# openai/blocksparse

Measured on AMD Instinct MI355X. Metric: bsmm_effective_tflops_4096x4096_bs32_d20, higher is better.
Workload: dtype bf16

## Files before the change

### blocksparse_amd/csrc/bsmm_updat_v2.h

```cpp
#pragma once
#include <type_traits>

#include "bsmm_common.h"
#include "bsmm_plan.h"
#include "bsmm_updat_tr.h"

namespace bsmm {

#ifndef U2_NT_PARTS
#define U2_NT_PARTS 1
#endif
#ifndef U2_MAX_SLICES
#define U2_MAX_SLICES 8
#endif
#ifndef U2_CH_ROWS
#define U2_CH_ROWS 16
#endif
#ifndef U2_SETB_FROM
#define U2_SETB_FROM 0
#endif
constexpr int U2_CH = U2_CH_ROWS;
constexpr int U2_KS = U2_CH / 16;
constexpr int U2_D = 64 / U2_CH;
constexpr int U2_AHEAD = U2_D / 2;
static_assert(U2_CH == 16 || U2_CH == 32, "chunk = 1 or 2 K-steps");
constexpr int u2_ring(int ws) { return ws == 32 ? 2 : U2_D; }
constexpr int u2_lds_bytes(int ws) { return u2_ring(ws) * 2 * U2_CH * ws * 64; }
constexpr int U2_CH0 = 32;
#ifndef U2_RING5
#define U2_RING5 0
#endif
constexpr int u2_lds_bytes0(int ws) { return U2_RING5 ? 5 * ws * 32 * (U2_CH0 * 2) : 131072; }

#ifdef U2_STAMPS
__device__ unsigned long long g_u2_trace[1024 * 8];
#define U2_STAMP(k, v) do { if (wave == 0 && lane == 0 && blockIdx.x < 1024) g_u2_trace[blockIdx.x * 8 + (k)] = (v); } while (0)
#else
#define U2_STAMP(k, v) do { } while (0)
#endif

__device__ __forceinline__ const void* uniform_ptr(const void* p) {
    const uint64_t v = reinterpret_cast<uint64_t>(p);
    const uint32_t lo = __builtin_amdgcn_readfirstlane((uint32_t)v), hi = __builtin_amdgcn_readfirstlane((uint32_t)(v >> 32));
    return reinterpret_cast<const void*>(((uint64_t)hi << 32) | lo);
}

__device__ __forceinline__ void glds16_saddr(const void* sbase, uint32_t voff, uint32_t lds_byte_addr) {
    unsigned keep;
    asm volatile("s_mov_b32 %0, m0\n\ts_mov_b32 m0, %3\n\ts_nop 0\n\tglobal_load_lds_dwordx4 %1, %2\n\ts_mov_b32 m0, %0"
                 : "=&s"(keep)
                 : "v"(voff), "s"(sbase), "s"(lds_byte_addr)
                 : "memory");
}
__device__ __forceinline__ void glds16_saddr_x2(const void* sbase, uint32_t voff0, uint32_t voff1, uint32_t lds_byte_addr) {
    unsigned keep;
    asm volatile("s_mov_b32 %0, m0\n\ts_mov_b32 m0, %4\n\ts_nop 0\n\tglobal_load_lds_dwordx4 %1, %3\n\t"
                 "s_add_u32 m0, m0, 0x400\n\ts_nop 0\n\tglobal_load_lds_dwordx4 %2, %3\n\ts_mov_b32 m0, %0"
                 : "=&s"(keep)
                 : "v"(voff0), "v"(voff1), "s"(sbase), "s"(lds_byte_addr)
                 : "memory", "scc");
}

__device__ __forceinline__ void glds16_saddr_x4(const void* sbase, uint32_t v0, uint32_t v1, uint32_t v2, uint32_t v3, uint32_t lds_byte_addr) {
    unsigned keep;
    asm volatile("s_mov_b32 %0, m0\n\ts_mov_b32 m0, %6\n\ts_nop 0\n\tglobal_load_lds_dwordx4 %1, %5\n\t"
                 "s_add_u32 m0, m0, 0x400\n\ts_nop 0\n\tglobal_load_lds_dwordx4 %2, %5\n\t"
                 "s_add_u32 m0, m0, 0x400\n\ts_nop 0\n\tglobal_load_lds_dwordx4 %3, %5\n\t"
                 "s_add_u32 m0, m0, 0x400\n\ts_nop 0\n\tglobal_load_lds_dwordx4 %4, %5\n\ts_mov_b32 m0, %0"
                 : "=&s"(keep)
                 : "v"(v0), "v"(v1), "v"(v2), "v"(v3), "s"(sbase), "s"(lds_byte_addr)
                 : "memory", "scc");
}

__device__ __forceinline__ const unsigned char* pick_ptr(const PtrList8& l, int idx) {
    const void* p = l.p[0];
#pragma unroll
    for (int k = 1; k < 8; ++k) p = (idx == k) ? l.p[k] : p;
    return static_cast<const unsigned char*>(p);
}

template <class DT, int LDSB>
__device__ __forceinline__ void u2_direct_block(const PtrList8& Xs, const PtrList8& Es, float* __restrict__ scratch, const int32_t* __restrict__ plan,
                                                int N, int Cf, int Kf, int pcount, int e, long region0, unsigned char* smem) {
    typedef typename DT::T T;
    constexpr int SLOT = 2048, D = LDSB / U2_WAVES / SLOT;
    static_assert(D >= 2 && LDSB >= U2_WAVES * 4096, "direct blocks: a ring of two chunks per wave and 64 KiB for the reduction");
    const int lane = threadIdx.x & 63;
    const int wave = __builtin_amdgcn_readfirstlane(threadIdx.x >> 6);
    const int DP = plan[30];
    const int d = e / DP, q = e - d * DP;
    const int32_t* de = plan + plan[29] + 4 * d;
    const int c = __builtin_amdgcn_readfirstlane(de[1]), k = __builtin_amdgcn_readfirstlane(de[2]);
    unsigned char* ring = smem + wave * (D * SLOT);
    const uint32_t ring_addr = lds_addr_of(ring);
    const int drow = lane >> 2, dpiece = lane & 3;
    const int g16 = lane >> 4, t16 = lane & 15, h = g16 >> 1;
    const int rd_base = (8 * h + (t16 >> 2)) * 64 + (16 * (g16 & 1) + 4 * (t16 & 3)) * 2;
    f32x16 acc;
#pragma unroll
    for (int i = 0; i < 16; ++i) acc[i] = 0.f;
    const int nch = (N + 15) >> 4;
    const int lo = (int)((long)nch * q / DP), hi = (int)((long)nch * (q + 1) / DP);
    const int first = lo + wave;
    const int myq = hi > first ? (hi - first + U2_WAVES - 1) / U2_WAVES : 0;
    for (int p = 0; p < pcount; ++p) {
        const T* X = reinterpret_cast<const T*>(pick_ptr(Xs, p)) + c * 32 + dpiece * 8;
        const T* E = reinterpret_cast<const T*>(pick_ptr(Es, p)) + k * 32 + dpiece * 8;
        auto issue = [&](int j, int pos) {
            const int r = min((first + U2_WAVES * j) * 16 + drow, N - 1);
            const uint32_t slot = __builtin_amdgcn_readfirstlane(ring_addr + pos * SLOT);
            glds16_asm(X + (size_t)r * Cf, slot);
            glds16_asm(E + (size_t)r * Kf, slot + 1024);
        };
#pragma unroll
        for (int j = 0; j < D - 1; ++j) issue(j, j);
        int rd_pos = 0, wr_pos = D - 1;
        for (int j = 0; j < myq; ++j) {
            issue(j + D - 1, wr_pos);
            asm volatile("s_waitcnt vmcnt(%0)" ::"n"(2 * (D - 1)) : "memory");
            const unsigned char* sp = ring + rd_pos * SLOT + rd_base;
            rd_pos = (rd_pos + 1 == D) ? 0 : rd_pos + 1;
            wr_pos = (wr_pos + 1 == D) ? 0 : wr_pos + 1;
            const uint2 a0 = ds_tr16(sp), a1 = ds_tr16(sp + 4 * 64), b0 = ds_tr16(sp + 1024), b1 = ds_tr16(sp + 1024 + 4 * 64);
            uint4 a = make_uint4(a0.x, a0.y, a1.x, a1.y);
            const uint4 b = make_uint4(b0.x, b0.y, b1.x, b1.y);
            const int nb = (first + U2_WAVES * j) * 16 + 8 * h;
            if (nb + 8 > N) {
                uint32_t* u = reinterpret_cast<uint32_t*>(&a);
#pragma unroll
                for (int i = 0; i < 4; ++i) u[i] &= ((nb + 2 * i < N) ? 0xffffu : 0u) | ((nb + 2 * i + 1 < N) ? 0xffff0000u : 0u);
            }
            asm volatile("s_waitcnt lgkmcnt(0)" ::: "memory");
            acc = DT::mfma32(a, b, acc);
        }
        asm volatile("s_waitcnt vmcnt(0)" ::: "memory");
    }
    __syncthreads();
    float* red = reinterpret_cast<float*>(smem);
#pragma unroll
    for (int reg = 0; reg < 16; ++reg) red[wave * 1024 + reg * 64 + lane] = acc[reg];
    __syncthreads();
    float sum = 0.f;
#pragma unroll
    for (int v = 0; v < U2_WAVES; ++v) sum += red[v * 1024 + threadIdx.x];
    const int reg = threadIdx.x >> 6, ln = threadIdx.x & 63;
    float* region = scratch + ((size_t)region0 * (U2_WAVES * U2_SLOTS) + (size_t)e) * 1024;
    region[((reg >> 2) * 64 + ln) * 4 + (reg & 3)] = sum;
}

template <class DT, int WS, int AXIS = 1>
__global__ void __launch_bounds__(64 * U2_WAVES, 4)
updat32_a1_v2_kernel(PtrList8 Xs, PtrList8 Es, typename DT::T* __restrict__ DW, float* __restrict__ scratch,
                     const int32_t* __restrict__ plan, int N, int Cf, int Kf, int pcount, float alpha, float beta, int flat, int main_grid, int rounds) {
    typedef typename DT::T T;
    static_assert(DT::is16 && (WS == 8 || WS == 16 || (WS == 32 && AXIS == 1)), "updat v2: 16-bit storage types, 8x8 / 16x16 windows (32x32: feature axis 1)");
    extern __shared__ __attribute__((aligned(16))) unsigned char smem[];
    constexpr int CH = AXIS == 1 ? U2_CH : U2_CH0;
    constexpr int KS = CH / 16;
    constexpr bool FIVE = AXIS == 0 && U2_RING5;
    constexpr int D = AXIS == 1 ? u2_ring(WS) : (WS == 16 ? 2 : 4);
    constexpr int AHEAD = D / 2;
    constexpr int ROWB = AXIS == 1 ? WS * 64 : CH * 2;
    constexpr int SLAB = AXIS == 1 ? CH * ROWB : WS * 32 * ROWB;
    constexpr int SLOT = 2 * SLAB;
    constexpr int PPR = ROWB / 16;
    constexpr int RPI = ROWB <= 1024 ? 1024 / ROWB : 1;
    constexpr int IPR = ROWB <= 1024 ? 1 : ROWB / 1024;
    constexpr int IPO = SLAB / 1024;
    constexpr int NI = 2 * IPO / U2_WAVES;
    static_assert((NI == 1 || NI == 2 || NI == 4) && NI * U2_WAVES == 2 * IPO && IPO % NI == 0, "the chunk must split evenly over the waves");

    const int mg = main_grid > 0 ? main_grid : (int)gridDim.x;
    if ((int)blockIdx.x >= mg) {
        if constexpr (AXIS == 1) u2_direct_block<DT, u2_lds_bytes(WS)>(Xs, Es, scratch, plan, N, Cf, Kf, pcount, (int)blockIdx.x - mg, (long)rounds * mg, smem);
        return;
    }
    const int lane = threadIdx.x & 63;
    const int wave = __builtin_amdgcn_readfirstlane(threadIdx.x >> 6);
    const int32_t* items = plan + plan[6];
    const int nchunks = (N + CH - 1) / CH;
    const int nfull = N / CH;
    const int CPI = pcount * nchunks;
    const bool xcd_mode = flat == 0 && (mg & 7) == 0;
    const int nsets = xcd_mode ? plan[8] : 1;
    const int nparts = xcd_mode ? 8 / nsets : 1;
    const int U = xcd_mode ? mg >> 3 : mg;
    const int xcd = xcd_mode ? (blockIdx.x & 7) : 0, uj = xcd_mode ? (blockIdx.x >> 3) : blockIdx.x;
    const int set = xcd / nparts, part = xcd - set * nparts;
    const int set_first = xcd_mode ? plan[9 + 2 * set] : 0, set_count = xcd_mode ? plan[10 + 2 * set] : plan[4];
    const int part_lo = (int)((long)part * CPI / nparts), part_hi = (int)((long)(part + 1) * CPI / nparts);
    const int full_rounds = set_count / U, m_last = set_count - full_rounds * U;
    const int k_last = m_last > 0 ? min(U / m_last, U2_MAX_SLICES) : 0;
    const int total_rounds = full_rounds + ((m_last > 0 && uj < m_last * k_last) ? 1 : 0);

    const uint32_t base_addr = lds_addr_of(smem);
    const int opE = (NI * wave) / IPO;
    const int ii0 = (NI * wave) % IPO;
    const int d_row0 = ROWB <= 1024 ? ii0 * RPI + lane / PPR : ii0 / IPR;
    auto row_of = [&](int q) -> int { return ROWB <= 1024 ? d_row0 + q * RPI : (ii0 + q) / IPR; };
    auto pos_of = [&](int q) -> int { return ROWB <= 1024 ? lane % PPR : ((ii0 + q) % IPR) * 64 + lane; };
    const uint32_t sub_off = ii0 * 1024;
    const uint32_t wave_off = (!FIVE ? opE * SLAB : 0) + sub_off;
    constexpr uint32_t HS = SLAB, RING0 = 5 * SLAB;
    const int F = opE ? Kf : Cf;
    const int my_piece0 = (lane % PPR) ^ ((d_row0 >> 2) & 3);
    const int g16 = lane >> 4, t16 = lane & 15;
    const int h = AXIS == 1 ? g16 >> 1 : lane >> 5;
    const int trow = t16 >> 2;
    const int tsub = (2 * (g16 & 1) + ((t16 & 3) >> 1)) * 16 + (t16 & 1) * 8;
    const int frag_row = AXIS == 1 ? (8 * h + trow) * ROWB + tsub : (lane & 31) * ROWB + ((h ^ (((lane & 31) >> 2) & 3)) << 4);
#ifdef U2_NO_PINGPONG
    const bool setb = false;
#else
    constexpr int SB = U2_SETB_FROM > 0 ? U2_SETB_FROM : ((WS == 8 && AXIS == 1) ? 4 : U2_WAVES / 2);
    const bool setb = wave >= SB;
#endif

    U2_STAMP(0, __builtin_amdgcn_s_memrealtime());
    U2_STAMP(4, (unsigned long long)total_rounds);
    for (int round = 0; round < total_rounds; ++round) {
        int item, r0, cnt;
        if (round < full_rounds) {
            item = set_first + round * U + uj;
            r0 = part_lo; cnt = part_hi - part_lo;
        } else {
            const int which = uj / k_last, slice = uj - which * k_last, L = part_hi - part_lo;
            item = set_first + full_rounds * U + which;
            r0 = part_lo + (int)((long)slice * L / k_last);
            cnt = part_lo + (int)((long)(slice + 1) * L / k_last) - r0;
        }
        if (cnt <= 0) continue;
        item = __builtin_amdgcn_readfirstlane(item);
        r0 = __builtin_amdgcn_readfirstlane(r0);
        cnt = __builtin_amdgcn_readfirstlane(cnt);
        const int32_t* it = items + (size_t)item * U2_ITEM;
        const int c0 = it[0], k0 = it[1];
        const int32_t* wd = it + 4 + wave * U2_WWORDS;
        const uint32_t meta = (uint32_t)__builtin_amdgcn_readfirstlane(wd[0]);
        const int n0 = meta & 15, n1 = (meta >> 4) & 15;

        auto piece_off = [&](int q) {
            const int row = row_of(q);
            if constexpr (AXIS == 1) {
                const int piece = pos_of(q) ^ (4 * (row & 3));
                const int col = min((opE ? k0 : c0) * 32 + piece * 8, F - 8);
                return (uint32_t)(row * F + col) * 2u;
            } else {
                const int piece = (lane % PPR) ^ ((row >> 2) & 3);
                const int feat = min((opE ? k0 : c0) * 32 + row, F - 1);
                return ((uint32_t)feat * (uint32_t)N + (uint32_t)piece * 8u) * 2u;
            }
        };
        const uint32_t voff0 = piece_off(0), voff1 = NI > 1 ? piece_off(1) : 0u, voff2 = NI > 2 ? piece_off(2) : 0u, voff3 = NI > 2 ? piece_off(3) : 0u;
        int aoff[2], boff[U2_SLOTS];
        if constexpr (AXIS == 1) {
            int c0i = (meta >> 8) & 15, c1i = (meta >> 12) & 15;
            if constexpr (WS == 32) {
                c0i |= (__builtin_amdgcn_readfirstlane(wd[1]) >> 29 & 1) << 4;
                c1i |= n1 > 0 ? (__builtin_amdgcn_readfirstlane(wd[1 + n0]) >> 29 & 1) << 4 : 0;
            }
            aoff[0] = frag_row + ((c0i ^ trow) << 6);
            aoff[1] = frag_row + ((c1i ^ trow) << 6);
#pragma unroll
            for (int j = 0; j < U2_SLOTS; ++j) {
                int ki = (meta >> (16 + 4 * j)) & 15;
                if constexpr (WS == 32) ki |= (__builtin_amdgcn_readfirstlane(wd[1 + j]) >> 30 & 1) << 4;
                boff[j] = SLAB + frag_row + ((ki ^ trow) << 6);
            }
        } else {
            aoff[0] = frag_row + (int)((meta >> 8) & 15) * (32 * ROWB);
            aoff[1] = frag_row + (int)((meta >> 12) & 15) * (32 * ROWB);
#pragma unroll
            for (int j = 0; j < U2_SLOTS; ++j) boff[j] = (FIVE ? 0 : SLAB) + frag_row + (int)((meta >> (16 + 4 * j)) & 15) * (32 * ROWB);
        }

        f32x16 acc[U2_SLOTS];
#pragma unroll
        for (int j = 0; j < U2_SLOTS; ++j)
#pragma unroll
            for (int i = 0; i < 16; ++i) acc[j][i] = 0.f;

        const uint32_t fstride = AXIS == 1 ? (uint32_t)(CH * F) * 2u : (uint32_t)CH * 2u;
        auto run = [&](auto n0_tag, auto n1_tag, auto setb_tag) {
            constexpr int N0 = decltype(n0_tag)::value, N1 = decltype(n1_tag)::value;
            constexpr bool SETB = decltype(setb_tag)::value;
            uint4 a0 = zero_u4(), a1 = zero_u4(), b[(N0 + N1) ? (N0 + N1) : 1];
#pragma unroll
            for (int j = 0; j < N0 + N1; ++j) b[j] = zero_u4();
            auto read_frags = [&](const unsigned char* slot, const unsigned char* slot_y, int ks) {
#ifdef U2_NO_READS
                asm volatile("" ::"s"(slot));
                return;
#endif
                if constexpr (AXIS == 1) {
                    slot += ks * 16 * ROWB;
                    {
                        const uint2 lo = ds_tr16(slot + aoff[0]), hi = ds_tr16(slot + aoff[0] + 4 * ROWB);
                        a0 = make_uint4(lo.x, lo.y, hi.x, hi.y);
                    }
                    if constexpr (N1 > 0) {
                        const uint2 lo = ds_tr16(slot + aoff[1]), hi = ds_tr16(slot + aoff[1] + 4 * ROWB);
                        a1 = make_uint4(lo.x, lo.y, hi.x, hi.y);
                    }
#pragma unroll
                    for (int j = 0; j < N0 + N1; ++j) {
                        const uint2 lo = ds_tr16(slot + boff[j]), hi = ds_tr16(slot + boff[j] + 4 * ROWB);
                        b[j] = make_uint4(lo.x, lo.y, hi.x, hi.y);
                    }
                } else {
                    a0 = *reinterpret_cast<const uint4*>(slot + (aoff[0] ^ (ks << 5)));
                    if constexpr (N1 > 0) a1 = *reinterpret_cast<const uint4*>(slot + (aoff[1] ^ (ks << 5)));
#pragma unroll
                    for (int j = 0; j < N0 + N1; ++j) b[j] = *reinterpret_cast<const uint4*>(slot_y + (boff[j] ^ (ks << 5)));
                }
            };
            auto multiply = [&]() {
#ifndef U2_NO_MFMA
#pragma unroll
                for (int j = 0; j < N0; ++j) acc[j] = DT::mfma32(a0, b[j], acc[j]);
                if constexpr (N1 > 0) {
#pragma unroll
                    for (int j = 0; j < N1; ++j) acc[N0 + j] = DT::mfma32(a1, b[N0 + j], acc[N0 + j]);
                }
#else
#pragma unroll
                for (int j = 0; j < N0 + N1; ++j) asm volatile("" ::"v"(b[j].x), "v"(b[j].y), "v"(b[j].z), "v"(b[j].w));
                asm volatile("" ::"v"(a0.x), "v"(a0.y), "v"(a0.z), "v"(a0.w));
                if constexpr (N1 > 0) asm volatile("" ::"v"(a1.x), "v"(a1.y), "v"(a1.z), "v"(a1.w));
#endif
            };
            const unsigned char* fb = nullptr;
            uint32_t rv0 = 0, rv1 = 0, rv2 = 0, rv3 = 0;
            int reg_left = 0, k_issue = 0;
#define U2_ISSUE_SLOW()                                                                                                      \
    do {                                                                                                                     \
        const int kk_ = min(k_issue, cnt - 1);                                                                               \
        const int g_ = r0 + kk_, p_ = __builtin_amdgcn_readfirstlane(g_ / nchunks), q_ = g_ - p_ * nchunks;                  \
        fb = static_cast<const unsigned char*>(uniform_ptr(opE ? pick_ptr(Es, p_) : pick_ptr(Xs, p_)));                      \
        const uint32_t dst_ = __builtin_amdgcn_readfirstlane(base_addr + wave_off + (!FIVE ? (uint32_t)(k_issue & (D - 1)) * SLOT : (uint32_t)((2 * k_issue + opE) % 5) * HS)); \
        uint32_t row_off_, sub0_, sub1_, sub2_, sub3_;                                                                       \
        if constexpr (AXIS == 1) {                                                        \
            row_off_ = (uint32_t)(q_ * CH * F) * 2u;                                                                         \
            sub0_ = (uint32_t)(max(0, q_ * CH + row_of(0) - (N - 1)) * F) * 2u;                                              \
            sub1_ = (uint32_t)(max(0, q_ * CH + row_of(1) - (N - 1)) * F) * 2u;                                              \
            sub2_ = (uint32_t)(max(0, q_ * CH + row_of(2) - (N - 1)) * F) * 2u;                                              \
            sub3_ = (uint32_t)(max(0, q_ * CH + row_of(3) - (N - 1)) * F) * 2u;                                              \
        } else {                                       \
            row_off_ = (uint32_t)(q_ * CH) * 2u;                                                                             \
            sub0_ = sub1_ = sub2_ = sub3_ = (uint32_t)max(0, q_ * CH + my_piece0 * 8 + 8 - N) * 2u;                          \
        }                                                                                                                    \
        U2_DMA1(fb, voff0 + row_off_ - sub0_, dst_);                                                                         \
        if constexpr (NI >= 2) U2_DMA1(fb, voff1 + row_off_ - sub1_, dst_ + 1024);                                           \
        if constexpr (NI == 4) U2_DMA1(fb, voff2 + row_off_ - sub2_, dst_ + 2048);                                           \
        if constexpr (NI == 4) U2_DMA1(fb, voff3 + row_off_ - sub3_, dst_ + 3072);                                           \
        rv0 = voff0 + row_off_ + fstride;                                                                                    \
        rv1 = voff1 + row_off_ + fstride;                                                                                    \
        rv2 = voff2 + row_off_ + fstride;                                                                                    \
        rv3 = voff3 + row_off_ + fstride;                                                                                    \
        reg_left = __builtin_amdgcn_readfirstlane(max(0, min(nfull - (q_ + 1), cnt - 1 - kk_)));                             \
        ++k_issue;                                                                                                           \
    } while (0)
#ifndef U2_NO_DMA
#define U2_DMA1(b_, v_, d_) glds16_saddr(b_, v_, d_)
#define U2_DMA2(b_, v0_, v1_, d_) glds16_saddr_x2(b_, v0_, v1_, d_)
#define U2_DMA4(b_, v0_, v1_, v2_, v3_, d_) glds16_saddr_x4(b_, v0_, v1_, v2_, v3_, d_)
#else
#define U2_DMA1(b_, v_, d_) asm volatile("" ::"v"(v_), "s"(d_), "s"(b_))
#define U2_DMA2(b_, v0_, v1_, d_) asm volatile("" ::"v"(v0_), "v"(v1_), "s"(d_), "s"(b_))
#define U2_DMA4(b_, v0_, v1_, v2_, v3_, d_) asm volatile("" ::"v"(v0_), "v"(v1_), "v"(v2_), "v"(v3_), "s"(d_), "s"(b_))
#endif
#define U2_ISSUE()                                                                                                           \
    do {                                                                                                                     \
        if (reg_left > 0) {                                                                                                  \
            --reg_left; ++k_issue;                                                                                           \
            if constexpr (NI == 4)      U2_DMA4(fb, rv0, rv1, rv2, rv3, ring_base + doff);                                       \
            else if constexpr (NI == 2) U2_DMA2(fb, rv0, rv1, ring_base + doff);                                                 \
            else                        U2_DMA1(fb, rv0, ring_base + doff);                                                      \
            rv0 += fstride;                                                                                                  \
            rv1 += fstride;                                                                                                  \
            if constexpr (NI == 4) { rv2 += fstride; rv3 += fstride; }                                                       \
        } else {                                                                                                             \
            U2_ISSUE_SLOW();                                                                                                 \
        }                                                                                                                    \
        if constexpr (!FIVE) doff = (doff + SLOT) & (D * SLOT - 1);                                                      \
        else { doff += 2 * HS; if (doff >= RING0) doff -= RING0; }                                                           \
    } while (0)
            k_issue = 0; reg_left = 0;
            if constexpr (!FIVE) {
#pragma unroll
                for (int d = 0; d < AHEAD; ++d) U2_ISSUE_SLOW();
            } else {
                U2_ISSUE_SLOW();
                if (!opE) U2_ISSUE_SLOW();
            }
            uint32_t vslot = !FIVE ? 0u : (uint32_t)HS;
            uint32_t vslot0 = 0;
            asm volatile("" : "+v"(vslot), "+v"(vslot0));
            uint32_t doff = !FIVE ? (uint32_t)AHEAD * SLOT : (uint32_t)((2 * k_issue + opE) % 5) * HS;
            const uint32_t ring_base = __builtin_amdgcn_readfirstlane(base_addr + wave_off);
            int cq = __builtin_amdgcn_readfirstlane(r0 - (r0 / nchunks) * nchunks);
#pragma unroll 1
            for (int i = 0; i < cnt; ++i) {
                if constexpr (!FIVE) {
                    asm volatile("s_waitcnt vmcnt(%0)" ::"n"(NI * AHEAD - NI) : "memory");
                } else {
                    if (opE) asm volatile("s_waitcnt vmcnt(0)" ::: "memory");
                    else     asm volatile("s_waitcnt vmcnt(%0)" ::"n"(NI) : "memory");
                }
                if (nfull != nchunks) {
                    if (cq == nfull) {
#pragma unroll
                        for (int e = 0; e < NI; ++e)
                            if (AXIS == 1 ? (cq * CH + row_of(e) >= N) : (cq * CH + my_piece0 * 8 >= N))
                                *reinterpret_cast<uint4*>(smem + (!FIVE ? (uint32_t)(i & (D - 1)) * SLOT : (uint32_t)((2 * i + opE) % 5) * HS) + wave_off + e * 1024 + lane * 16) = zero_u4();
                        asm volatile("s_waitcnt lgkmcnt(0)" ::: "memory");
                    }
                    if (++cq == nchunks) cq = 0;
                }
                if constexpr ((D == 2 || FIVE) && SETB) asm volatile("s_waitcnt lgkmcnt(0)" ::: "memory");
#ifndef U2_NO_BARRIER
                __builtin_amdgcn_s_barrier();
#endif
                const unsigned char* slot = smem + (!FIVE ? vslot : vslot0);
                const unsigned char* slot_y = smem + vslot;
                if constexpr (N0 == 0) {
                    U2_ISSUE();
                } else if constexpr (!SETB) {
                    read_frags(slot, slot_y, 0);
                    U2_ISSUE();
                    multiply();
#pragma unroll
                    for (int ks = 1; ks < KS; ++ks) { read_frags(slot, slot_y, ks); multiply(); }
                } else {
                    multiply();
                    __builtin_amdgcn_sched_barrier(0);
                    U2_ISSUE();
#pragma unroll
                    for (int ks = 0; ks < KS - 1; ++ks) { read_frags(slot, slot_y, ks); multiply(); }
                    read_frags(slot, slot_y, KS - 1);
                }
                if constexpr (!FIVE) {
                    vslot = (vslot + SLOT) & (D * SLOT - 1);
                } else {
                    vslot += 2 * HS;  vslot = vslot >= RING0 ? vslot - RING0 : vslot;
                    vslot0 += 2 * HS; vslot0 = vslot0 >= RING0 ? vslot0 - RING0 : vslot0;
                }
            }
#undef U2_ISSUE
#undef U2_ISSUE_SLOW
#undef U2_DMA1
#undef U2_DMA2
#undef U2_DMA4
            if constexpr (SETB && N0 > 0) multiply();
            asm volatile("s_waitcnt vmcnt(0)" ::: "memory");
            __builtin_amdgcn_s_barrier();
        };
        using std::integral_constant;
#define RUN(A, B)                                                                                                          \
    do {                                                                                                                   \
        if (setb) run(integral_constant<int, A>{}, integral_constant<int, B>{}, integral_constant<bool, true>{});          \
        else      run(integral_constant<int, A>{}, integral_constant<int, B>{}, integral_constant<bool, false>{});         \
    } while (0)
        switch (n0 * 8 + n1) {
            case 0 * 8 + 0: RUN(0, 0); break;
            case 1 * 8 + 0: RUN(1, 0); break;
            case 1 * 8 + 1: RUN(1, 1); break;
            case 1 * 8 + 2: RUN(1, 2); break;
            case 1 * 8 + 3: RUN(1, 3); break;
            case 2 * 8 + 0: RUN(2, 0); break;
            case 2 * 8 + 1: RUN(2, 1); break;
            case 2 * 8 + 2: RUN(2, 2); break;
            case 3 * 8 + 0: RUN(3, 0); break;
            case 3 * 8 + 1: RUN(3, 1); break;
            default:        RUN(4, 0); break;
        }
#undef RUN
        if (round == 0) { U2_STAMP(1, __builtin_amdgcn_s_memrealtime()); U2_STAMP(5, (unsigned long long)cnt); }

        if (scratch != nullptr) {
            float4* reg_base = reinterpret_cast<float4*>(scratch) + ((size_t)(round * mg + blockIdx.x) * (U2_WAVES * U2_SLOTS) + wave * U2_SLOTS) * 256 + lane;
#pragma unroll
            for (int j = 0; j < U2_SLOTS; ++j) {
                if (j >= n0 + n1) break;
#ifdef U2_NO_EPILOGUE
                if (alpha != 12345.f) continue;
#endif
#pragma unroll
                for (int q = 0; q < 4; ++q)
                {
#if U2_NT_PARTS
                    typedef float f4v __attribute__((ext_vector_type(4)));
                    const f4v v = {acc[j][4 * q + 0], acc[j][4 * q + 1], acc[j][4 * q + 2], acc[j][4 * q + 3]};
                    __builtin_nontemporal_store(v, reinterpret_cast<f4v*>(reg_base + (j * 4 + q) * 64));
#else
                    reg_base[(j * 4 + q) * 64] = make_float4(acc[j][4 * q + 0], acc[j][4 * q + 1], acc[j][4 * q + 2], acc[j][4 * q + 3]);
#endif
                }
            }
        } else {
#pragma unroll
            for (int j = 0; j < U2_SLOTS; ++j) {
                if (j >= n0 + n1) break;
                const int wid = __builtin_amdgcn_readfirstlane(wd[1 + j]) & 0x1fffffff;
                const size_t base = (size_t)wid * 1024 + (lane & 31);
#pragma unroll
                for (int reg = 0; reg < 16; ++reg) {
                    const int ci = (reg & 3) + 8 * (reg >> 2) + 4 * (lane >> 5);
                    const size_t idx = base + ci * 32;
#ifdef U2_NO_EPILOGUE
                    if (alpha == 12345.f) DW[idx] = DT::from_f32(acc[j][reg]);
                    continue;
#endif
                    float out = alpha * acc[j][reg];
                    if (beta != 0.f) out += beta * DT::to_f32(DW[idx]);
                    DW[idx] = DT::from_f32(out);
                }
            }
        }
        if (round == 0) U2_STAMP(2, __builtin_amdgcn_s_memrealtime());
    }
    U2_STAMP(3, __builtin_amdgcn_s_memrealtime());
}

__device__ __forceinline__ float4 u2_ld(const float4* p) {
#if U2_NT_PARTS
    typedef float f4v __attribute__((ext_vector_type(4)));
    const f4v v = __builtin_nontemporal_load(reinterpret_cast<const f4v*>(p));
    return make_float4(v.x, v.y, v.z, v.w);
#else
    return *p;
#endif
}

template <class DT, bool SUMS>
__global__ void __launch_bounds__(128)
updat2_reduce_kernel(const float* __restrict__ parts, typename DT::T* __restrict__ DW, float* __restrict__ sums, const int32_t* __restrict__ plan,
                     const int32_t* __restrict__ bmap, const float* __restrict__ gate, int direct_region0, int main_grid, int flat, int CPI, float alpha, float beta, int q64 = 0) {
    const int w = blockIdx.x;
    const int qq = threadIdx.x >> 6, l = threadIdx.x & 63;
    const int32_t bm = bmap[w];
    const bool direct = bm <= -2;
    const int item = direct ? 0 : bm >> 8, slot = direct ? 0 : bm & 255;
    const bool xcd_mode = flat == 0 && (main_grid & 7) == 0;
    const int nsets = xcd_mode ? plan[8] : 1;
    const int nparts = xcd_mode ? 8 / nsets : 1;
    const int U = xcd_mode ? main_grid >> 3 : main_grid;
    int set = 0;
    if (xcd_mode)
        for (int s = 1; s < nsets; ++s) if (item >= plan[9 + 2 * s]) set = s;
    const int set_first = xcd_mode ? plan[9 + 2 * set] : 0, set_count = xcd_mode ? plan[10 + 2 * set] : plan[4];
    const int pos = item - set_first;
    const int full_rounds = set_count / U, m_last = set_count - full_rounds * U;
    const int k_last = m_last > 0 ? min(U / m_last, U2_MAX_SLICES) : 0;
    const float4* base = reinterpret_cast<const float4*>(parts) + ((size_t)slot * 4 + qq) * 64 + l;
    constexpr size_t REGION = (size_t)U2_WAVES * U2_SLOTS * 256;
    const bool sliced = pos >= full_rounds * U;
    const int which = pos - full_rounds * U;
    const float4 zero4 = make_float4(0.f, 0.f, 0.f, 0.f);
    float4 acc0 = zero4, acc1 = zero4;
    auto part_len = [&](int part) -> int {
        const unsigned part_lo = (unsigned)part * (unsigned)CPI / (unsigned)nparts, part_hi = (unsigned)(part + 1) * (unsigned)CPI / (unsigned)nparts;
        return (int)(part_hi - part_lo);
    };
    auto add = [](float4& a, const float4& v) { a.x += v.x; a.y += v.y; a.z += v.z; a.w += v.w; };
    if (direct) {
        const int dp = plan[30];
        const float4* p0 = base + (size_t)direct_region0 * REGION + (size_t)((-2 - bm) * dp) * 256;
        float4 v0[8], v1[8];
#pragma unroll
        for (int part = 0; part < 8; ++part) {
            v0[part] = v1[part] = zero4;
            if (part < dp) { v0[part] = u2_ld(p0 + (size_t)part * 256); v1[part] = u2_ld(p0 + (size_t)part * 256 + 128); }
        }
#pragma unroll
        for (int part = 0; part < 8; ++part) { add(acc0, v0[part]); add(acc1, v1[part]); }
    } else if (!sliced) {
        const int round = pos / U, uj = pos - round * U;
        float4 v0[8], v1[8];
#pragma unroll
        for (int part = 0; part < 8; ++part) {
            v0[part] = v1[part] = zero4;
            if (part < nparts && part_len(part) > 0) {
                const int xcd = set * nparts + part;
                const float4* p = base + ((size_t)round * main_grid + (xcd_mode ? uj * 8 + xcd : uj)) * REGION;
                v0[part] = u2_ld(p); v1[part] = u2_ld(p + 128);
            }
        }
#pragma unroll
        for (int part = 0; part < 8; ++part) { add(acc0, v0[part]); add(acc1, v1[part]); }
    } else {
        for (int part = 0; part < nparts; ++part) {
            const int L = part_len(part);
            if (L <= 0) continue;
            const int xcd = set * nparts + part;
            const float4* rb = base + (size_t)full_rounds * main_grid * REGION;
            auto where = [&](int slice) -> const float4* {
                if (slice >= k_last) return nullptr;
                if (L < k_last) {
                    const unsigned lo = (unsigned)slice * (unsigned)L / (unsigned)k_last, hi = (unsigned)(slice + 1) * (unsigned)L / (unsigned)k_last;
                    if (hi == lo) return nullptr;
                }
                const int uj = which * k_last + slice;
                return rb + (size_t)(xcd_mode ? uj * 8 + xcd : uj) * REGION;
            };
            for (int sl = 0; sl < k_last; sl += 8) {
                float4 a[8], b[8];
#pragma unroll
                for (int e = 0; e < 8; ++e) {
                    const float4* p = where(sl + e);
                    a[e] = b[e] = zero4;
                    if (p) { a[e] = u2_ld(p); b[e] = u2_ld(p + 128); }
                }
#pragma unroll
                for (int e = 0; e < 8; ++e) { add(acc0, a[e]); add(acc1, b[e]); }
            }
        }
    }
#pragma unroll
    for (int hq = 0; hq < 2; ++hq) {
        const int q = qq + 2 * hq;
        const float4 acc = hq ? acc1 : acc0;
        const float r[4] = {acc.x, acc.y, acc.z, acc.w};
        const int row = 8 * q + 4 * (l >> 5), col = l & 31;
        const size_t o = q64 ? (size_t)(w >> 2) * 4096 + (size_t)(32 * ((w >> 1) & 1) + row) * 64 + 32 * (w & 1) + col : (size_t)w * 1024 + (size_t)row * 32 + col;
        const int ostep = q64 ? 64 : 32;
        if constexpr (SUMS) {
#pragma unroll
            for (int e = 0; e < 4; ++e) sums[o + e * ostep] = r[e];
        } else {
            const float a = gate ? alpha * gate[q64 ? w >> 2 : w] : alpha;
#pragma unroll
            for (int e = 0; e < 4; ++e) {
                float v = a * r[e];
                if (beta != 0.f) v += beta * DT::to_f32(DW[o + e * ostep]);
                DW[o + e * ostep] = DT::from_f32(v);
            }
        }
    }
}

template <class DT>
__global__ void __launch_bounds__(256)
updat_finalize_gated_kernel(const float* __restrict__ scratch, typename DT::T* __restrict__ DW, size_t n, int bsq, float alpha, float beta,
                            const float* __restrict__ gate, const int32_t* __restrict__ skip_if = nullptr) {
    const size_t i = ((size_t)blockIdx.x * 256 + threadIdx.x) * 4;
    if (i >= n || (skip_if && skip_if[0] != 0)) return;
    const float4 s = *reinterpret_cast<const float4*>(scratch + i);
    const float a = gate ? alpha * gate[i / bsq] : alpha;
    float v[4] = {a * s.x, a * s.y, a * s.z, a * s.w};
    if (beta != 0.f) {
#pragma unroll
        for (int e = 0; e < 4; ++e) v[e] += beta * DT::to_f32(DW[i + e]);
    }
#pragma unroll
    for (int e = 0; e < 4; ++e) DW[i + e] = DT::from_f32(v[e]);
}

}
```

Measured before the change: 668.6.

## Add unrolled steady-state loop with immediate-offset LDS DMA and reads

Adds a fast path for the AXIS==1, KS==1 update loop that unrolls the ring of chunk intervals 2 or 4 times. It uses compile-time immediate offsets for the global-to-LDS DMA (m0 set from the base plus an immediate) and for the ds_read_tr16 fragment reads, and toggles the address high bits with XOR. The aim is to cut per-iteration scalar and vector address arithmetic and loop overhead in the main pipelined loop. The remaining iterations and the tail still go through the existing generic loop. This adds complexity and preconditions (alignment, no partial chunks), and changes register pressure.

```diff
diff --git a/blocksparse_amd/csrc/bsmm_updat_v2.h b/blocksparse_amd/csrc/bsmm_updat_v2.h
--- a/blocksparse_amd/csrc/bsmm_updat_v2.h
+++ b/blocksparse_amd/csrc/bsmm_updat_v2.h
@@ -19,6 +19,10 @@
 #ifndef U2_SETB_FROM
 #define U2_SETB_FROM 0
 #endif
+#ifndef U2_UNROLL
+#define U2_UNROLL 4
+#endif
+static_assert(U2_UNROLL == 0 || U2_UNROLL == 2 || U2_UNROLL == 4, "unrolled steady state: 2 or 4 intervals per body, 0 = off");
 constexpr int U2_CH = U2_CH_ROWS;
 constexpr int U2_KS = U2_CH / 16;
 constexpr int U2_D = 64 / U2_CH;
@@ -70,6 +74,36 @@
                  : "=&s"(keep)
                  : "v"(v0), "v"(v1), "v"(v2), "v"(v3), "s"(sbase), "s"(lds_byte_addr)
                  : "memory", "scc");
+}
+
+template <uint32_t IMM>
+__device__ __forceinline__ void glds16_m0(const void* sbase, uint32_t voff, uint32_t lds_base) {
+    asm volatile("s_add_u32 m0, %2, %3\n\ts_nop 0\n\tglobal_load_lds_dwordx4 %0, %1"
+                 :
+                 : "v"(voff), "s"(sbase), "s"(lds_base), "n"(IMM)
+                 : "memory", "scc", "m0");
+}
+template <uint32_t IMM>
+__device__ __forceinline__ void glds16_m0_x2(const void* sbase, uint32_t voff0, uint32_t voff1, uint32_t lds_base) {
+    asm volatile("s_add_u32 m0, %3, %4\n\ts_nop 0\n\tglobal_load_lds_dwordx4 %0, %2\n\t"
+                 "s_add_u32 m0, m0, 0x400\n\ts_nop 0\n\tglobal_load_lds_dwordx4 %1, %2"
+                 :
+                 : "v"(voff0), "v"(voff1), "s"(sbase), "s"(lds_base), "n"(IMM)
+                 : "memory", "scc", "m0");
+}
+template <uint32_t IMM>
+__device__ __forceinline__ void glds16_m0_x4(const void* sbase, uint32_t v0, uint32_t v1, uint32_t v2, uint32_t v3, uint32_t lds_base) {
+    asm volatile("s_add_u32 m0, %5, %6\n\ts_nop 0\n\tglobal_load_lds_dwordx4 %0, %4\n\t"
+                 "s_add_u32 m0, m0, 0x400\n\ts_nop 0\n\tglobal_load_lds_dwordx4 %1, %4\n\t"
+                 "s_add_u32 m0, m0, 0x400\n\ts_nop 0\n\tglobal_load_lds_dwordx4 %2, %4\n\t"
+                 "s_add_u32 m0, m0, 0x400\n\ts_nop 0\n\tglobal_load_lds_dwordx4 %3, %4"
+                 :
+                 : "v"(v0), "v"(v1), "v"(v2), "v"(v3), "s"(sbase), "s"(lds_base), "n"(IMM)
+                 : "memory", "scc", "m0");
+}
+__device__ __forceinline__ uint2 ds_tr16_at(uint32_t lds_byte_addr) {
+    s16x4 v = __builtin_amdgcn_ds_read_tr16_b64_v4i16((__attribute__((address_space(3))) s16x4*)(uintptr_t)lds_byte_addr);
+    return __builtin_bit_cast(uint2, v);
 }
 
 __device__ __forceinline__ const unsigned char* pick_ptr(const PtrList8& l, int idx) {
@@ -284,9 +318,14 @@
         auto run = [&](auto n0_tag, auto n1_tag, auto setb_tag) {
             constexpr int N0 = decltype(n0_tag)::value, N1 = decltype(n1_tag)::value;
             constexpr bool SETB = decltype(setb_tag)::value;
+#pragma unroll
+            for (int j = 0; j < N0 + N1; ++j) asm volatile("" : "+v"(acc[j]));
             uint4 a0 = zero_u4(), a1 = zero_u4(), b[(N0 + N1) ? (N0 + N1) : 1];
 #pragma unroll
             for (int j = 0; j < N0 + N1; ++j) b[j] = zero_u4();
+            int ao0 = aoff[0], ao1 = aoff[1], bo[(N0 + N1) ? (N0 + N1) : 1];
+#pragma unroll
+            for (int j = 0; j < N0 + N1; ++j) bo[j] = boff[j];
             auto read_frags = [&](const unsigned char* slot, const unsigned char* slot_y, int ks) {
 #ifdef U2_NO_READS
                 asm volatile("" ::"s"(slot));
@@ -295,23 +334,23 @@
                 if constexpr (AXIS == 1) {
                     slot += ks * 16 * ROWB;
                     {
-                        const uint2 lo = ds_tr16(slot + aoff[0]), hi = ds_tr16(slot + aoff[0] + 4 * ROWB);
+                        const uint2 lo = ds_tr16(slot + ao0), hi = ds_tr16(slot + ao0 + 4 * ROWB);
                         a0 = make_uint4(lo.x, lo.y, hi.x, hi.y);
                     }
                     if constexpr (N1 > 0) {
-                        const uint2 lo = ds_tr16(slot + aoff[1]), hi = ds_tr16(slot + aoff[1] + 4 * ROWB);
+                        const uint2 lo = ds_tr16(slot + ao1), hi = ds_tr16(slot + ao1 + 4 * ROWB);
                         a1 = make_uint4(lo.x, lo.y, hi.x, hi.y);
                     }
 #pragma unroll
                     for (int j = 0; j < N0 + N1; ++j) {
-                        const uint2 lo = ds_tr16(slot + boff[j]), hi = ds_tr16(slot + boff[j] + 4 * ROWB);
+                        const uint2 lo = ds_tr16(slot + bo[j]), hi = ds_tr16(slot + bo[j] + 4 * ROWB);
                         b[j] = make_uint4(lo.x, lo.y, hi.x, hi.y);
                     }
                 } else {
-                    a0 = *reinterpret_cast<const uint4*>(slot + (aoff[0] ^ (ks << 5)));
-                    if constexpr (N1 > 0) a1 = *reinterpret_cast<const uint4*>(slot + (aoff[1] ^ (ks << 5)));
-#pragma unroll
-                    for (int j = 0; j < N0 + N1; ++j) b[j] = *reinterpret_cast<const uint4*>(slot_y + (boff[j] ^ (ks << 5)));
+                    a0 = *reinterpret_cast<const uint4*>(slot + (ao0 ^ (ks << 5)));
+                    if constexpr (N1 > 0) a1 = *reinterpret_cast<const uint4*>(slot + (ao1 ^ (ks << 5)));
+#pragma unroll
+                    for (int j = 0; j < N0 + N1; ++j) b[j] = *reinterpret_cast<const uint4*>(slot_y + (bo[j] ^ (ks << 5)));
                 }
             };
             auto multiply = [&]() {
@@ -393,14 +432,140 @@
                 U2_ISSUE_SLOW();
                 if (!opE) U2_ISSUE_SLOW();
             }
-            uint32_t vslot = !FIVE ? 0u : (uint32_t)HS;
+            const uint32_t ring_base = __builtin_amdgcn_readfirstlane(base_addr + wave_off);
+            int cq = __builtin_amdgcn_readfirstlane(r0 - (r0 / nchunks) * nchunks);
+            int i0 = 0;
+#if U2_UNROLL > 0
+            if constexpr (AXIS == 1 && !FIVE && KS == 1 && WS != 32) {
+                constexpr int UNR = U2_UNROLL < D ? U2_UNROLL : D;
+                static_assert(UNR == D || (2 * UNR == D && AHEAD == UNR), "a body is the whole ring or half of it");
+                constexpr uint32_t T = UNR < D ? (uint32_t)UNR * SLOT : 0u;
+                static_assert(((UNR - 1) * SLOT & 0xffff) + 4 * ROWB < 0x10000, "slot offset + second read fit the offset field");
+                if (cq + cnt <= nfull && cnt - AHEAD >= UNR && (base_addr & (uint32_t)(D * SLOT - 1)) == 0u) {
+                    const int nbody = (cnt - AHEAD) / UNR;
+                    uint32_t fa0 = base_addr + (uint32_t)ao0, fa1 = base_addr + (uint32_t)ao1, fbo[(N0 + N1) ? (N0 + N1) : 1];
+                    asm volatile("" : "+v"(fa0));
+                    if constexpr (N1 > 0) asm volatile("" : "+v"(fa1));
+#pragma unroll
+                    for (int j = 0; j < N0 + N1; ++j) { fbo[j] = base_addr + (uint32_t)bo[j]; asm volatile("" : "+v"(fbo[j])); }
+                    uint32_t dring = ring_base ^ T;
+                    asm volatile("" : "+s"(dring));
+#define U2_VADD(v_, s_) asm volatile("v_add_u32_e32 %0, %1, %0" : "+v"(v_) : "s"(s_))
+#define U2_VXOR(v_, c_) asm volatile("v_xor_b32_e32 %0, %1, %0" : "+v"(v_) : "n"(c_))
+#ifndef U2_NO_DMA
+#define U2_FDMA(J)                                                                                                           \
+    do {                                                                                                                     \
+        constexpr uint32_t dimm_ = UNR == D ? (uint32_t)(((J) + AHEAD) % D) * SLOT : (uint32_t)(J) * SLOT;                   \
+        if constexpr (NI == 4)      glds16_m0_x4<dimm_>(fb, rv0, rv1, rv2, rv3, dring);                                      \
+        else if constexpr (NI == 2) glds16_m0_x2<dimm_>(fb, rv0, rv1, dring);                                                \
+        else                        glds16_m0<dimm_>(fb, rv0, dring);                                                        \
+          \
+                                                                                     \
+        U2_VADD(rv0, fstride);                                                                                               \
+        if constexpr (NI >= 2) U2_VADD(rv1, fstride);                                                                        \
+        if constexpr (NI == 4) { U2_VADD(rv2, fstride); U2_VADD(rv3, fstride); }                                             \
+    } while (0)
+#else
+#define U2_FDMA(J)                                                                                                           \
+    do {                                                                                                                     \
+        asm volatile("" ::"v"(rv0), "v"(rv1), "s"(dring), "s"(fb));                                                          \
+        U2_VADD(rv0, fstride);                                                                                               \
+        U2_VADD(rv1, fstride);                                                                                               \
+    } while (0)
+#endif
+#ifndef U2_NO_READS
+#define U2_FREAD(J)                                                                                                          \
+    do {                                                                                                                     \
+        constexpr uint32_t im_ = ((uint32_t)(J) * SLOT) & 0xffffu;                                                           \
+        {                                                                                                                    \
+            const uint2 lo_ = ds_tr16_at(fa0 + im_), hi_ = ds_tr16_at(fa0 + (im_ + 4 * ROWB));                               \
+            a0 = make_uint4(lo_.x, lo_.y, hi_.x, hi_.y);                                                                     \
+        }                                                                                                                    \
+        if constexpr (N1 > 0) {                                                                                              \
+            const uint2 lo_ = ds_tr16_at(fa1 + im_), hi_ = ds_tr16_at(fa1 + (im_ + 4 * ROWB));                               \
+            a1 = make_uint4(lo_.x, lo_.y, hi_.x, hi_.y);                                                                     \
+        }                                                                                                                    \
+        _Pragma("unroll") for (int j_ = 0; j_ < N0 + N1; ++j_) {                                                             \
+            const uint2 lo_ = ds_tr16_at(fbo[j_] + im_), hi_ = ds_tr16_at(fbo[j_] + (im_ + 4 * ROWB));                       \
+            b[j_] = make_uint4(lo_.x, lo_.y, hi_.x, hi_.y);                                                                  \
+        }                                                                                                                    \
+    } while (0)
+#else
+#define U2_FREAD(J) asm volatile("" ::"v"(fa0))
+#endif
+#define U2_FTOGGLE(J)                                                                                                        \
+    do {                                                                                                                     \
+        constexpr uint32_t rj_ = ((uint32_t)(J) * SLOT) & ~0xffffu;                                                          \
+        constexpr uint32_t rn_ = (J) + 1 < UNR ? ((uint32_t)((J) + 1) * SLOT) & ~0xffffu : T;                                \
+        if constexpr ((rj_ ^ rn_) != 0u && N0 > 0) {                                                                         \
+            U2_VXOR(fa0, rj_ ^ rn_);                                                                                         \
+            if constexpr (N1 > 0) U2_VXOR(fa1, rj_ ^ rn_);                                                                   \
+            _Pragma("unroll") for (int j_ = 0; j_ < N0 + N1; ++j_) U2_VXOR(fbo[j_], rj_ ^ rn_);                              \
+        }                                                                                                                    \
+    } while (0)
+#ifndef U2_NO_BARRIER
+#define U2_FBARRIER() __builtin_amdgcn_s_barrier()
+#else
+#define U2_FBARRIER() do { } while (0)
+#endif
+#define U2_FINTERVAL(J)                                                                                                      \
+    do {                                                                                                                     \
+        asm volatile("s_waitcnt vmcnt(%0)" ::"n"(NI * AHEAD - NI) : "memory");         \
+        if constexpr (D == 2 && SETB) asm volatile("s_waitcnt lgkmcnt(0)" ::: "memory");         \
+        U2_FBARRIER();                                                                                   \
+        if constexpr (N0 == 0) {                                                                                             \
+            U2_FDMA(J);                                                                                                      \
+        } else if constexpr (!SETB) {                                                                                        \
+            U2_FREAD(J);                                                                                                     \
+              \
+                                                \
+            __builtin_amdgcn_sched_barrier(0);                                                                               \
+            U2_FDMA(J);                                                                                                      \
+            __builtin_amdgcn_sched_barrier(0);                                               \
+            multiply();                                                                                                      \
+        } else {                                                                                                             \
+            multiply();                                                                                                      \
+            __builtin_amdgcn_sched_barrier(0);                                                                               \
+            U2_FDMA(J);                                                                                                      \
+            U2_FREAD(J);                                                                                                     \
+        }                                                                                                                    \
+        U2_FTOGGLE(J);                                                                                                       \
+         \
+                                            \
+        __builtin_amdgcn_sched_barrier(0);                                                                                   \
+    } while (0)
+#pragma unroll 1
+                    for (int g = 0; g < nbody; ++g) {
+                        U2_FINTERVAL(0);
+                        U2_FINTERVAL(1);
+                        if constexpr (UNR == 4) {
+                            U2_FINTERVAL(2);
+                            U2_FINTERVAL(3);
+                        }
+                        if constexpr (T != 0u) { dring ^= T; asm volatile("" : "+s"(dring)); }
+                    }
+#undef U2_FINTERVAL
+#undef U2_FBARRIER
+#undef U2_FTOGGLE
+#undef U2_FREAD
+#undef U2_FDMA
+#undef U2_VXOR
+#undef U2_VADD
+                    i0 = nbody * UNR;
+                    k_issue += i0; reg_left -= i0; cq += i0;
+                    const uint32_t back = base_addr + ((nbody & 1) ? T : 0u);
+                    ao0 = (int)(fa0 - back); ao1 = (int)(fa1 - back);
+#pragma unroll
+                    for (int j = 0; j < N0 + N1; ++j) bo[j] = (int)(fbo[j] - back);
+                }
+            }
+#endif
+            uint32_t vslot = !FIVE ? (uint32_t)(i0 & (D - 1)) * SLOT : (uint32_t)HS;
             uint32_t vslot0 = 0;
             asm volatile("" : "+v"(vslot), "+v"(vslot0));
-            uint32_t doff = !FIVE ? (uint32_t)AHEAD * SLOT : (uint32_t)((2 * k_issue + opE) % 5) * HS;
-            const uint32_t ring_base = __builtin_amdgcn_readfirstlane(base_addr + wave_off);
-            int cq = __builtin_amdgcn_readfirstlane(r0 - (r0 / nchunks) * nchunks);
+            uint32_t doff = !FIVE ? (uint32_t)((i0 + AHEAD) & (D - 1)) * SLOT : (uint32_t)((2 * k_issue + opE) % 5) * HS;
 #pragma unroll 1
-            for (int i = 0; i < cnt; ++i) {
+            for (int i = i0; i < cnt; ++i) {
                 if constexpr (!FIVE) {
                     asm volatile("s_waitcnt vmcnt(%0)" ::"n"(NI * AHEAD - NI) : "memory");
                 } else {
```

New measurement: 668.5, median of 2. About the same (-0.0%).
